# GPUs/goVideoCompressor

Hardware: AMD Instinct MI355X
Metric: encoded frames/sec (whole node), 1080p30->H.264 CRF23 (higher is better)
Workload: dtype uint8 (8-bit 4:2:0 samples, int32 transforms)

## Files before the change

csrc/kernels/bindings_hip.cc:

```cpp
#include <pybind11/pybind11.h>
#include <pybind11/stl.h>

#include <cstdint>
#include <stdexcept>
#include <vector>

#include "../common/hevc_ctu_coder.h"
#include "hevc_decode.h"
#include "route.h"

namespace py = pybind11;

extern "C" {
long long mivc_hevc_entropy_state_bytes(int W, int H);
int mivc_launch_hevc_entropy(const void* pic, int B, const int* qp, const void* ctu, const void* cu, const void* col,
                             const unsigned long long* nzmap, const int16_t* cy, const int16_t* cb, const int16_t* cr,
                             uint8_t* state, long long state_bytes, uint8_t* out, unsigned cap, unsigned* sizes,
                             int* errs, unsigned long long* offs, unsigned long long* offs_host, uint8_t* dst,
                             unsigned long long dst_cap, int* overflow, void* stream, unsigned long long* prof,
                             int* gprog, void* gctx, const unsigned long long* tsmap);
long long mivc_hevc_entropy_ctx_bytes();
int mivc_launch_hevc_tskip_probe(int nblk, const uint16_t* src, const uint16_t* pred, int16_t* lev, uint16_t* rec, int* flag,
                                 long long* terms, int bd, int qp, int intra, int dst, int scan, int sdh, int rdoq,
                                 int rdoq_lam, int lamq, void* stream);
// ... 71 lines not shown
void mivc_launch_wp_stats16(const uint16_t* y, const uint16_t* u, const uint16_t* v, int w, int h, int npics,
                            unsigned long long* out, void* stream);
void mivc_launch_wp_stats(const uint8_t* y, const uint8_t* u, const uint8_t* v, int w, int h, int npics,
                          unsigned long long* out, void* stream);
void mivc_launch_wp_src(const uint8_t* src, uint8_t* dst, const int* wt, int B, long long plane_bytes, void* stream);
void mivc_launch_p_part8(int B, int wmb, int hmb, const uint8_t* src_y, const uint8_t* ref, const uint8_t* hp,
                         const int16_t* mv, const int16_t* pm, int* cost, uint8_t* pred, int16_t* mv8, const int* qp,
                         const int8_t* aq, int overhead, int min_satd, void* stream, const void* route, int nbuf,
                         const int* bits16, const uint8_t* dir16);
void mivc_launch_encode_intra(int B, int wmb, int hmb, const uint8_t* src_y, const uint8_t* src_u,
                              const uint8_t* src_v, uint8_t* rec_y, uint8_t* rec_u, uint8_t* rec_v, const int* qp,
                              int chroma_qp_offset, void* hdr, int16_t* coef, uint8_t* nz,
                              const uint8_t* intra_flag, const int* intra_count, int* err, int use_i4x4,
                              const int8_t* aq, void* stream, int use_i8x8, const void* route, int nbuf,
                              int slice_rows, int trellis, float trellis_lambda, int* gprog, long long gprog_ints);
void mivc_launch_deblock(int B, int wmb, int hmb, uint8_t* rec_y, uint8_t* rec_u, uint8_t* rec_v, const void* hdr,
                         const uint8_t* nz, int chroma_qp_offset, int alpha_off, int beta_off, int* err,
                         void* stream, const void* route, int nbuf);
void mivc_launch_decode_picture_dpb(int B, int wmb, int hmb, int dpb_n, uint8_t* dpb_y, uint8_t* dpb_u, uint8_t* dpb_v,
                                    const int16_t* cur_idx, const int16_t* reftab, const int16_t* wp, const int16_t* sub,
                                    const void* hdr, const uint32_t* mask, const uint32_t* off,
                                    const int16_t* coef, const int8_t* run, int any_inter, int chroma_qp_offset,
                                    uint8_t* nz, int* err, void* stream);
void mivc_launch_deblock_dpb(int B, int wmb, int hmb, int dpb_n, uint8_t* dpb_y, uint8_t* dpb_u, uint8_t* dpb_v,
                             const int16_t* cur_idx, const void* hdr, const uint8_t* nz, const uint8_t* bs,
                             int chroma_qp_offset, int alpha_off, int beta_off, int* err, void* stream);
void mivc_launch_decode_picture_dpb16(int B, int wmb, int hmb, int dpb_n, uint16_t* dpb_y, uint16_t* dpb_u,
                                      uint16_t* dpb_v, const int16_t* cur_idx, const int16_t* reftab, const int16_t* wp,
                                      const int16_t* sub, const void* hdr, const uint32_t* mask, const uint32_t* off,
                                      const int16_t* coef, const int8_t* run, int any_inter, int chroma_qp_offset, int bd,
                                      uint8_t* nz, int* err, void* stream);
void mivc_launch_deblock_dpb16(int B, int wmb, int hmb, int dpb_n, uint16_t* dpb_y, uint16_t* dpb_u, uint16_t* dpb_v,
                               const int16_t* cur_idx, const void* hdr, const uint8_t* bs, int chroma_qp_offset,
// ... 377 lines not shown
                           uintptr_t ru, uintptr_t rv, uintptr_t qp, int cqo, uintptr_t hdr, uintptr_t coef,
                           uintptr_t nz, uintptr_t intra_flag, uintptr_t intra_count, uintptr_t err, int use_i4x4,
                           uintptr_t stream, uintptr_t aq, int use_i8x8, uintptr_t route, int nbuf, int slice_rows,
                           int trellis, float trellis_lambda, uintptr_t gprog, long long gprog_ints) {
    mivc_launch_encode_intra(B, wmb, hmb, P<uint8_t>(sy), P<uint8_t>(su), P<uint8_t>(sv), P<uint8_t>(ry),
                             P<uint8_t>(ru), P<uint8_t>(rv), P<int>(qp), cqo, P<void>(hdr), P<int16_t>(coef),
                             P<uint8_t>(nz), P<uint8_t>(intra_flag), P<int>(intra_count), P<int>(err), use_i4x4,
                             P<int8_t>(aq), S(stream), use_i8x8, P<void>(route), nbuf, slice_rows, trellis,
                             trellis_lambda, P<int>(gprog), gprog_ints);
  }, py::arg("B"), py::arg("wmb"), py::arg("hmb"), py::arg("sy"), py::arg("su"), py::arg("sv"), py::arg("ry"),
     py::arg("ru"), py::arg("rv"), py::arg("qp"), py::arg("cqo"), py::arg("hdr"), py::arg("coef"), py::arg("nz"),
     py::arg("intra_flag"), py::arg("intra_count"), py::arg("err"), py::arg("use_i4x4"), py::arg("stream"),
     py::arg("aq") = 0, py::arg("use_i8x8") = 0, py::arg("route") = 0, py::arg("nbuf") = 0, py::arg("slice_rows") = 0,
     py::arg("trellis") = 0, py::arg("trellis_lambda") = 1.0f, py::arg("gprog") = 0, py::arg("gprog_ints") = 0);
  m.def("deblock", [](int B, int wmb, int hmb, uintptr_t ry, uintptr_t ru, uintptr_t rv, uintptr_t hdr, uintptr_t nz,
                      int cqo, int alpha_off, int beta_off, uintptr_t err, uintptr_t stream, uintptr_t route, int nbuf) {
    mivc_launch_deblock(B, wmb, hmb, P<uint8_t>(ry), P<uint8_t>(ru), P<uint8_t>(rv), P<void>(hdr), P<uint8_t>(nz),
                        cqo, alpha_off, beta_off, P<int>(err), S(stream), P<void>(route), nbuf);
  }, py::arg("B"), py::arg("wmb"), py::arg("hmb"), py::arg("ry"), py::arg("ru"), py::arg("rv"), py::arg("hdr"),
     py::arg("nz"), py::arg("cqo"), py::arg("alpha_off"), py::arg("beta_off"), py::arg("err"), py::arg("stream"),
     py::arg("route") = 0, py::arg("nbuf") = 0);
  m.def("decode_picture_dpb", [](int B, int wmb, int hmb, int dpb_n, uintptr_t y, uintptr_t u, uintptr_t v,
                                 uintptr_t cur_idx, uintptr_t reftab, uintptr_t wp, uintptr_t sub,
                                 uintptr_t hdr, uintptr_t mask, uintptr_t off, uintptr_t coef, uintptr_t run,
                                 int any_inter, int cqo, uintptr_t nz, uintptr_t err, uintptr_t stream) {
    if (dpb_n < 1 || dpb_n > 32767) throw std::invalid_argument("decode_picture_dpb: dpb_n must be 1..32767");
    mivc_launch_decode_picture_dpb(B, wmb, hmb, dpb_n, P<uint8_t>(y), P<uint8_t>(u), P<uint8_t>(v), P<int16_t>(cur_idx),
                                   P<int16_t>(reftab), P<int16_t>(wp), P<int16_t>(sub), P<void>(hdr),
                                   P<uint32_t>(mask), P<uint32_t>(off), P<int16_t>(coef), P<int8_t>(run), any_inter,
                                   cqo, P<uint8_t>(nz), P<int>(err), S(stream));
  });
  m.def("deblock_dpb", [](int B, int wmb, int hmb, int dpb_n, uintptr_t y, uintptr_t u, uintptr_t v, uintptr_t cur_idx,
                          uintptr_t hdr, uintptr_t nz, uintptr_t bs, int cqo, int alpha_off, int beta_off, uintptr_t err,
                          uintptr_t stream) {
    if (dpb_n < 1 || dpb_n > 32767) throw std::invalid_argument("deblock_dpb: dpb_n must be 1..32767");
    mivc_launch_deblock_dpb(B, wmb, hmb, dpb_n, P<uint8_t>(y), P<uint8_t>(u), P<uint8_t>(v), P<int16_t>(cur_idx),
// ... 437 lines not shown
```

csrc/kernels/deblock.hip:

```cpp
#include "kcommon.h"

namespace mivc {
namespace gpu {

using h264::MbHeader;

struct DeblockArgs {
  Geom g;
  uint8_t *rec_y, *rec_u, *rec_v;
  const MbHeader* hdr;
  const uint8_t* nz;
  int chroma_qp_offset;
  int alpha_off, beta_off;
  int* err;
  const uint8_t* bs_in;
  int dpb_n;
  const int16_t* cur_idx;
  const SlotRoute* rt;
  int nbuf;
};

constexpr int kDeblockWaves = 16;
constexpr int kRing = 8;
constexpr int kRingU = 4;
constexpr int LT = 20;
constexpr int CT = 12;
constexpr int kSlotWords = 24;
constexpr int kMaxCols = 480;

struct DeblockShared {
  alignas(16) uint8_t ty[LT * LT];
  alignas(16) uint8_t tc[2][CT * CT];
  alignas(16) uint32_t hdrw[3][12];
  uint32_t nzw[3][4];
  int bs[2][4][4];
  int par[2][2][2][5];
  uint32_t left_y[16];
  uint32_t left_c[2][8];
  uint32_t bot_y[4][3];
  uint32_t bot_c[2][2];
};

struct DeblockTables {
  int alpha[52], beta[52], tc0[52][3], cqp[52];
};

__device__ __forceinline__ void filt(uint32_t& P, uint32_t& Q, int bs, int alpha, int beta, int tc0, bool chroma) {
  const int p3 = __builtin_amdgcn_ubfe(P, 0, 8), p2 = __builtin_amdgcn_ubfe(P, 8, 8);
  const int p1 = __builtin_amdgcn_ubfe(P, 16, 8), p0 = __builtin_amdgcn_ubfe(P, 24, 8);
  const int q0 = __builtin_amdgcn_ubfe(Q, 0, 8), q1 = __builtin_amdgcn_ubfe(Q, 8, 8);
// ... 17 lines not shown
    const bool sp = apb && strong, sq = aqb && strong;
    np0 = sp ? (p2 + 2 * p1 + 2 * p0 + 2 * q0 + q1 + 4) >> 3 : (2 * p1 + p0 + q1 + 2) >> 2;
    np1 = sp ? (p2 + p1 + p0 + q0 + 2) >> 2 : p1;
    np2 = sp ? (2 * p3 + 3 * p2 + p1 + p0 + q0 + 4) >> 3 : p2;
    nq0 = sq ? (p1 + 2 * p0 + 2 * q0 + 2 * q1 + q2 + 4) >> 3 : (2 * q1 + q0 + p1 + 2) >> 2;
    nq1 = sq ? (p0 + q0 + q1 + q2 + 2) >> 2 : q1;
    nq2 = sq ? (2 * q3 + 3 * q2 + q1 + q0 + p0 + 4) >> 3 : q2;
  }
  if (on) {
    const int pv[4] = {p3, np2, np1, np0}, qv[4] = {nq0, nq1, nq2, q3};
    P = pack4_u8(pv);
    Q = pack4_u8(qv);
  }
}

__device__ __forceinline__ void edges4(uint32_t (&d)[5], const DeblockShared& S, int dir, int line, bool chroma,
                                       bool has_nb) {
  const int seg = chroma ? (line >> 1) : (line >> 2);
#pragma unroll
  for (int e = 0; e < 4; ++e) {
    int bs = S.bs[dir][e][seg & 3];
    if (e == 0 && !has_nb) bs = 0;
    if (chroma && (e & 1)) bs = 0;
    const int* P = S.par[dir][e == 0 ? 0 : 1][chroma ? 1 : 0];
    const int tc0 = P[2 + (bs > 0 && bs < 4 ? bs - 1 : 0)];
    filt(d[e], d[e + 1], bs, P[0], P[1], tc0, chroma);
  }
}

__global__ __launch_bounds__(64 * kDeblockWaves) void deblock_wavefront(DeblockArgs a) {
  __shared__ DeblockShared SS[kDeblockWaves][2];
  __shared__ uint32_t ringL[kDeblockWaves - 1][kRing][kSlotWords];
  __shared__ uint32_t ringB[kMaxCols][kSlotWords];
  __shared__ uint32_t ringU[kDeblockWaves][kRingU][kSlotWords];
  __shared__ int prog[kMaxRows];
  __shared__ DeblockTables T;
  const Geom& g = a.g;
  const int slot = blockIdx.x;
  if (a.rt && (a.rt[slot].kind < 0 || !(a.rt[slot].flags & SF_DEBLOCK))) return;
  for (int i = threadIdx.x; i < g.hmb; i += blockDim.x) prog[i] = 0;
  for (int i = threadIdx.x; i < 52; i += blockDim.x) {
    T.alpha[i] = h264::kAlpha[i];
    T.beta[i] = h264::kBeta[i];
    T.tc0[i][0] = h264::kTc0[i][0];
    T.tc0[i][1] = h264::kTc0[i][1];
    T.tc0[i][2] = h264::kTc0[i][2];
    T.cqp[i] = h264::kChromaQp[i];
  }
  __syncthreads();
  const int w = wave_id();
  auto opaque_lane = []() { int l = lane_id(); asm volatile("" : "+v"(l)); return l; };
  const int half = lane_id() >> 5;
  DeblockShared& S = SS[w][half];
#define DB_LANE_VALUES                                                     \
  const int lane = opaque_lane(), hl = lane & 31;                          \
  const bool is_c = hl >= 16;  \
  const int ccomp = (hl - 16) >> 3, cline = hl & 7;                        \
  const int line = is_c ? cline : hl;
  const int W = g.W, cw = g.cw(), wmb = g.wmb, hmb = g.hmb;
  const size_t pic = a.dpb_n ? static_cast<size_t>(slot) * a.dpb_n + a.cur_idx[slot]
                             : route_index(a.rt, a.nbuf, slot, RO_CUR);
  uint8_t* recy = a.rec_y + pic * g.ysize();
  uint8_t* const rcu = a.rec_u + pic * g.csize();
  uint8_t* const rcv = a.rec_v + pic * g.csize();
  const uint8_t* bs_in = a.bs_in ? a.bs_in + static_cast<size_t>(slot) * g.nmb() * 16 : nullptr;
  auto recc = [&](int c) { return c ? rcv : rcu; };
  const uint32_t* hdr32 = reinterpret_cast<const uint32_t*>(a.hdr) + static_cast<size_t>(slot) * g.nmb() * 16;
  const uint32_t* nz32 = reinterpret_cast<const uint32_t*>(a.nz) + static_cast<size_t>(slot) * g.nmb() * 4;

  auto load_inputs = [&](int x, int y, uint32_t (&v)[5]) {
    DB_LANE_VALUES
    (void)line;
    const uint8_t* a1 = recy + static_cast<size_t>(y * 16 + (hl & 15)) * W + x * 16;
    const uint8_t* a2 = a1 + 8;
    if (is_c) a1 = a2 = recc(ccomp) + static_cast<size_t>(y * 8 + cline) * cw + x * 8;
    const size_t mb = static_cast<size_t>(y) * wmb + x;
    const size_t mbt = y > 0 ? mb - wmb : mb;
    const uint32_t* a3 = hl < 12 ? hdr32 + mb * 16 + hl
                                 : (hl < 24 ? hdr32 + mbt * 16 + (hl - 12)
                                            : (hl < 28 ? nz32 + mb * 4 + (hl - 24) : nz32 + mbt * 4 + (hl - 28)));
    const uint2 q1 = *reinterpret_cast<const uint2*>(a1);
    const uint2 q2 = *reinterpret_cast<const uint2*>(a2);
    v[0] = q1.x; v[1] = q1.y; v[2] = q2.x; v[3] = q2.y;
    v[4] = *a3;
  };

  for (int yu = 2 * w; yu < hmb; yu += 2 * kDeblockWaves) {
    const int yl = yu + 1;
    const int y = half ? yl : yu;
    const bool row_ok = y < hmb;
    const bool last_row = y == hmb - 1;
    const bool has_top = y > 0;
    if (half && w < kDeblockWaves - 1 && yl >= 2 * kDeblockWaves && row_ok && (lane_id() & 31) == 0)
      row_wait_lds(prog, yl - 2 * kDeblockWaves + 1, wmb, a.err);
    uint32_t nxt[5] = {0, 0, 0, 0, 0};
    if (!half) load_inputs(0, y, nxt);
    for (int step = 0; step < wmb + 2; ++step) {
      const int x = half ? step - 2 : step;
      const bool act = row_ok && x >= 0 && x < wmb;
      DB_LANE_VALUES
      const uint32_t cur[5] = {nxt[0], nxt[1], nxt[2], nxt[3], nxt[4]};
      if (row_ok && x + 1 >= 0 && x + 1 < wmb) load_inputs(x + 1, y, nxt);
      if (act) {
        const bool has_left = x > 0, last_col = x == wmb - 1;
        {
          uint32_t* dst = hl < 12 ? &S.hdrw[0][hl]
                                  : (hl < 24 ? &S.hdrw[2][hl - 12] : (hl < 28 ? &S.nzw[0][hl - 24] : &S.nzw[2][hl - 28]));
          *dst = cur[4];
        }
        wave_sync();
        const MbHeader* HQ = reinterpret_cast<const MbHeader*>(S.hdrw[0]);
        {
          const int dir = hl >> 4, e = (hl >> 2) & 3, k = hl & 3;
          int bs = 0;
          const bool mbedge = e == 0;
          if (bs_in) {
            bs = (bs_in[(static_cast<size_t>(y) * wmb + x) * 16 + (hl >> 1)] >> ((hl & 1) * 4)) & 15;
          } else if (!mbedge || (dir == 0 ? has_left : has_top)) {
            const int pw = mbedge ? (dir == 0 ? 1 : 2) : 0;
            const MbHeader* HP = reinterpret_cast<const MbHeader*>(S.hdrw[pw]);
            const uint8_t* nzbp = reinterpret_cast<const uint8_t*>(S.nzw[pw]);
            const uint8_t* nzb0 = reinterpret_cast<const uint8_t*>(S.nzw[0]);
            const int rq = dir == 0 ? (e + 4 * k) : (k + 4 * e);
            const int rp = dir == 0 ? (mbedge ? 3 + 4 * k : e - 1 + 4 * k) : (mbedge ? k + 12 : k + 4 * (e - 1));
            const bool iq = h264::mbk_is_intra(HQ->kind), ip = h264::mbk_is_intra(HP->kind);
            if ((e & 1) && (HQ->flags & h264::MBF_T8x8)) bs = 0;
            else if (mbedge && (iq || ip)) bs = 4;
            else if (iq || ip) bs = 3;
            else if (nzbp[rp] || nzb0[rq]) bs = 2;
            else {
              const int qp_ = ((rp >> 3) & 1) * 2 + ((rp & 3) >> 1), qq_ = ((rq >> 3) & 1) * 2 + ((rq & 3) >> 1);
              bool diff = false;
#pragma unroll
              for (int l = 0; l < 2; ++l) {
                const int fp = HP->ref[l][qp_], fq = HQ->ref[l][qq_];
                if ((fp >= 0) != (fq >= 0) || (fp >= 0 && fp != fq)) {
                  diff = true;
                } else if (fp >= 0) {
                  const int dx = HP->mv[l][qp_][0] - HQ->mv[l][qq_][0], dy = HP->mv[l][qp_][1] - HQ->mv[l][qq_][1];
                  diff |= dx >= 4 || dx <= -4 || dy >= 4 || dy <= -4;
                }
              }
              bs = diff ? 1 : 0;
            }
          }
          S.bs[dir][e][k] = bs;
        }
        if (hl < 8) {
          const int dir = hl >> 2, inner = (hl >> 1) & 1, ch = hl & 1;
          const int qpq = HQ->qp;
          const int qpn = reinterpret_cast<const MbHeader*>(S.hdrw[dir == 0 ? 1 : 2])->qp;
          int qq = qpq, qn = inner ? qpq : qpn;
          if (ch) {
            qq = T.cqp[clampi(qq + a.chroma_qp_offset, 0, 51)];
            qn = T.cqp[clampi(qn + a.chroma_qp_offset, 0, 51)];
          }
          const int qpav = (qq + qn + 1) >> 1;
          const int ia = clampi(qpav + a.alpha_off, 0, 51), ib = clampi(qpav + a.beta_off, 0, 51);
          int* P = S.par[dir][inner][ch];
          P[0] = T.alpha[ia];
          P[1] = T.beta[ib];
          P[2] = T.tc0[ia][0];
          P[3] = T.tc0[ia][1];
          P[4] = T.tc0[ia][2];
        }
        if (has_top) {
          if (!half) row_wait_lds(prog, y - 1, min(x + 2, wmb), a.err);
          if (hl < kSlotWords) {
            const uint32_t v = half ? ringU[w][x % kRingU][hl]
                                    : (w == 0 ? ringB[x][hl] : ringL[w - 1][x % kRing][hl]);
            if (hl < 16) *reinterpret_cast<uint32_t*>(&S.ty[(hl >> 2) * LT + 4 + (hl & 3) * 4]) = v;
            else {
              const int c = (hl - 16) >> 2, r = ((hl - 16) >> 1) & 1, h = hl & 1;
              *reinterpret_cast<uint32_t*>(&S.tc[c][(2 + r) * CT + 4 + h * 4]) = v;
            }
          }
        }
        wave_sync();

        uint32_t d[5];
        if (!is_c) {
          d[0] = has_left ? S.left_y[hl] : 0u;
          d[1] = cur[0]; d[2] = cur[1]; d[3] = cur[2]; d[4] = cur[3];
        } else {
          d[0] = has_left ? S.left_c[ccomp][cline] : 0u;
          d[1] = cur[0]; d[2] = cur[0]; d[3] = cur[1]; d[4] = 0u;
        }
        edges4(d, S, 0, line, is_c, has_left);
        if (!is_c) {
          uint32_t* row = reinterpret_cast<uint32_t*>(&S.ty[(hl + 4) * LT]);
          row[0] = d[0]; row[1] = d[1]; row[2] = d[2]; row[3] = d[3]; row[4] = d[4];
        } else {
          uint32_t* row = reinterpret_cast<uint32_t*>(&S.tc[ccomp][(cline + 4) * CT]);
          row[0] = d[0];
          row[1] = (d[1] & 0x00FFFFFFu) | (d[2] & 0xFF000000u);
          row[2] = d[3];
        }
        wave_sync();

        {
          uint8_t* col = is_c ? &S.tc[ccomp][4 + cline] : &S.ty[4 + hl];
          const int pitch = is_c ? CT : LT;
          const int nw = is_c ? 3 : 5;
          uint32_t c[5] = {0, 0, 0, 0, 0};
#pragma unroll
          for (int k = 0; k < 5; ++k) {
            if (k < nw) {
              int v4[4];
#pragma unroll
              for (int r = 0; r < 4; ++r) v4[r] = col[(4 * k + r) * pitch];
              c[k] = pack4_u8(v4);
            }
          }
          if (is_c) { c[4] = 0; c[3] = c[2]; c[2] = c[1]; }
          edges4(c, S, 1, line, is_c, has_top);
          if (is_c) { c[1] = (c[1] & 0x00FFFFFFu) | (c[2] & 0xFF000000u); c[2] = c[3]; }
#pragma unroll
          for (int k = 0; k < 5; ++k) {
            if (k < nw && (k > 0 || has_top)) {
#pragma unroll
              for (int r = 0; r < 4; ++r) col[(4 * k + r) * pitch] = static_cast<uint8_t>(c[k] >> (8 * r));
            }
          }
        }
        wave_sync();

        {
          const int r = hl & 15;
          const bool rowok = r <= 12 || last_row;
          if (!is_c) {
            if (rowok) {
              const uint8_t* t = &S.ty[(r + 4) * LT + 4];
              uint32_t* o = reinterpret_cast<uint32_t*>(recy + static_cast<size_t>(y * 16 + r) * W + x * 16);
              const uint32_t* ti = reinterpret_cast<const uint32_t*>(t);
              o[0] = ti[0]; o[1] = ti[1]; o[2] = ti[2];
              if (last_col) o[3] = ti[3];
            }
          } else if (rowok && has_left) {
            *reinterpret_cast<uint32_t*>(recy + static_cast<size_t>(y * 16 + r) * W + x * 16 - 4) =
                *reinterpret_cast<const uint32_t*>(&S.ty[(r + 4) * LT]);
          }
          if (hl < 3) {
            if (has_top) {
              const uint32_t* ti = reinterpret_cast<const uint32_t*>(&S.ty[(1 + hl) * LT + 4]);
              uint32_t* o = reinterpret_cast<uint32_t*>(recy + static_cast<size_t>(y * 16 - 3 + hl) * W + x * 16);
              o[0] = ti[0]; o[1] = ti[1]; o[2] = ti[2]; o[3] = ti[3];
            }
          } else if (hl < 5) {
            if (has_top) {
              const int c = hl - 3;
              const uint32_t* ti = reinterpret_cast<const uint32_t*>(&S.tc[c][3 * CT + 4]);
              uint32_t* o = reinterpret_cast<uint32_t*>(recc(c) + static_cast<size_t>(y * 8 - 1) * cw + x * 8);
              o[0] = ti[0]; o[1] = ti[1];
            }
          } else if (hl >= 16) {
            const int c = (hl - 16) >> 3, rc = hl & 7;
            if (rc <= 6 || last_row) {
              const uint32_t* ti = reinterpret_cast<const uint32_t*>(&S.tc[c][(rc + 4) * CT]);
              uint32_t* o = reinterpret_cast<uint32_t*>(recc(c) + static_cast<size_t>(y * 8 + rc) * cw + x * 8);
              o[0] = ti[1];
              if (last_col) o[1] = ti[2];
              if (has_left) o[-1] = ti[0];
            }
          }
        }

        if (!last_row && hl < kSlotWords) {
          uint32_t vp, vc;
          if (hl < 16) {
            const int r = hl >> 2, k = hl & 3;
            vp = k < 3 ? S.bot_y[r][k] : *reinterpret_cast<const uint32_t*>(&S.ty[(r + 16) * LT]);
            vc = *reinterpret_cast<const uint32_t*>(&S.ty[(r + 16) * LT + 4 + 4 * k]);
          } else {
            const int c = (hl - 16) >> 2, r = ((hl - 16) >> 1) & 1, h = hl & 1;
            vp = h == 0 ? S.bot_c[c][r] : *reinterpret_cast<const uint32_t*>(&S.tc[c][(r + 10) * CT]);
            vc = *reinterpret_cast<const uint32_t*>(&S.tc[c][(r + 10) * CT + 4 + 4 * h]);
          }
// ... 13 lines not shown
            }
            if (last_col) {
              if (x >= kRing) row_wait_lds(prog, y + 1, x + 1 - kRing, a.err);
              ringL[w][x % kRing][hl] = vc;
            }
          } else {
            if (has_left) ringU[w][(x - 1) % kRingU][hl] = vp;
            if (last_col) ringU[w][x % kRingU][hl] = vc;
          }
        }
        wave_sync();
        if (!is_c) S.left_y[hl] = *reinterpret_cast<const uint32_t*>(&S.ty[(hl + 4) * LT + 16]);
        else S.left_c[ccomp][cline] = *reinterpret_cast<const uint32_t*>(&S.tc[ccomp][(cline + 4) * CT + 8]);
        if (hl < 12) S.bot_y[hl / 3][hl % 3] = *reinterpret_cast<const uint32_t*>(&S.ty[(hl / 3 + 16) * LT + 4 + 4 * (hl % 3)]);
        else if (hl < 16) { const int i = hl - 12; S.bot_c[i >> 1][i & 1] = *reinterpret_cast<const uint32_t*>(&S.tc[i >> 1][((i & 1) + 10) * CT + 4]); }
        else if (hl < 28) S.hdrw[1][hl - 16] = S.hdrw[0][hl - 16];
        else S.nzw[1][hl - 28] = S.nzw[0][hl - 28];
        wave_sync();
        __builtin_amdgcn_fence(__ATOMIC_RELEASE, "workgroup", "local");
        if (hl == 0) __hip_atomic_store(prog + y, x + 1, __ATOMIC_RELAXED, __HIP_MEMORY_SCOPE_WORKGROUP);
      }
    }
  }
}

}
}

using namespace mivc::gpu;

extern "C" void mivc_launch_deblock(int B, int wmb, int hmb, uint8_t* rec_y, uint8_t* rec_u, uint8_t* rec_v,
                                    const void* hdr, const uint8_t* nz, int chroma_qp_offset, int alpha_off,
                                    int beta_off, int* err, void* stream, const void* route, int nbuf) {
  DeblockArgs a;
  a.rt = static_cast<const SlotRoute*>(route);
  a.nbuf = nbuf;
  a.g = Geom{B, wmb, hmb, wmb * 16, hmb * 16};
  a.rec_y = rec_y;
  a.rec_u = rec_u;
  a.rec_v = rec_v;
  a.hdr = static_cast<const mivc::h264::MbHeader*>(hdr);
  a.nz = nz;
  a.chroma_qp_offset = chroma_qp_offset;
  a.alpha_off = alpha_off;
  a.beta_off = beta_off;
  a.err = err;
  a.bs_in = nullptr;
  a.dpb_n = 0;
  a.cur_idx = nullptr;
  hipLaunchKernelGGL(deblock_wavefront, dim3(B), dim3(64 * kDeblockWaves), 0, static_cast<hipStream_t>(stream), a);
}

extern "C" void mivc_launch_deblock_dpb(int B, int wmb, int hmb, int dpb_n, uint8_t* dpb_y, uint8_t* dpb_u,
                                        uint8_t* dpb_v, const int16_t* cur_idx, const void* hdr, const uint8_t* nz,
                                        const uint8_t* bs, int chroma_qp_offset, int alpha_off, int beta_off, int* err,
                                        void* stream) {
  DeblockArgs a;
  a.rt = nullptr;
  a.nbuf = 0;
  a.g = Geom{B, wmb, hmb, wmb * 16, hmb * 16};
  a.rec_y = dpb_y;
  a.rec_u = dpb_u;
  a.rec_v = dpb_v;
  a.hdr = static_cast<const mivc::h264::MbHeader*>(hdr);
  a.nz = nz;
  a.chroma_qp_offset = chroma_qp_offset;
  a.alpha_off = alpha_off;
  a.beta_off = beta_off;
  a.err = err;
  a.bs_in = bs;
  a.dpb_n = dpb_n;
  a.cur_idx = cur_idx;
  hipLaunchKernelGGL(deblock_wavefront, dim3(B), dim3(64 * kDeblockWaves), 0, static_cast<hipStream_t>(stream), a);
}
```

govideocompressor_amd/models/h264_gpu.py:

```python
from __future__ import annotations

import concurrent.futures as cf
import math
import os
import time
from dataclasses import dataclass

import numpy as np
import torch

from ..ops import native
from .gop import PicPlan, col_to_list0, dpb_frames, fixed_types, gop_plan, h264_plan

MB_HDR_BYTES = 64
NO_COST = 0x3FFFFFFF
ROUTE_DTYPE = np.dtype([("kind", "i1"), ("cur", "i1"), ("n0", "i1"), ("l1", "i1"), ("l0", "i1", (4,)),
                        ("w1", "<i2", (4,)), ("dsf", "<i2", (4,)), ("dcopy", "i1", (4,)), ("flags", "u1"),
                        ("col_l1", "i1"), ("disp", "<i2")])
assert ROUTE_DTYPE.itemsize == 32
COL_NONE = -128


def col_map_row(cur: PicPlan, col: PicPlan) -> np.ndarray:
    return np.array([[COL_NONE if m is None else m - r for r, m in enumerate(row)] for row in col_to_list0(cur, col)],
# ... 260 lines not shown
        self.src = planes()
        self.nb = params.eff_bframes()
        self.nref = params.eff_refs()
        self.nref_frames = dpb_frames(self.nref, params.eff_pyramid(), self.nb)
        self.nbuf = self.nref_frames + 2
        NB = self.nbuf
        self.rec_pool = (torch.zeros((B, NB, H, W), dtype=u8, device=dev),
                         torch.zeros((B, NB, H // 2, W // 2), dtype=u8, device=dev),
                         torch.zeros((B, NB, H // 2, W // 2), dtype=u8, device=dev))
        self.rec = [tuple(p[:, i] for p in self.rec_pool) for i in range(NB)]
        self.hp_bytes = 3 * (H + 8) * (W + 8)
        self.hp_pool = torch.empty(B * NB * self.hp_bytes + 64, dtype=u8, device=dev)
        self.hdr = [torch.zeros((B, nmb, MB_HDR_BYTES), dtype=u8, device=dev) for _ in range(2)]
        self.coef = [torch.zeros((B, nmb, COEF_PER_MB), dtype=i16, device=dev) for _ in range(2)]
        self.nz = torch.zeros((B, nmb, 16), dtype=u8, device=dev)
        self.mv = torch.zeros((B, nmb, 2), dtype=i16, device=dev)
        self.mv_tmp = torch.zeros((B, nmb, 2), dtype=i16, device=dev)
        self.mv8 = torch.zeros((B, nmb, 4, 2), dtype=i16, device=dev)
        self.prev_mv = torch.zeros((B, nmb, 2), dtype=i16, device=dev)
        self.me_cost = torch.zeros((B, nmb), dtype=i32, device=dev)
        self.intra_cost = torch.zeros((B, nmb), dtype=i32, device=dev)
        self.pred = torch.zeros((B, nmb, 256), dtype=u8, device=dev)
        self.mref = torch.zeros((B, nmb), dtype=torch.int8, device=dev)
        self.dref = torch.zeros((B, nmb, 4), dtype=torch.int8, device=dev)
        self.seed = [torch.zeros((B, nmb, 2), dtype=i16, device=dev) for _ in range(2)]
        self._slot_ar = torch.arange(B, device=dev)
        if self.nref > 1:
            K = self.nref - 1
            self.xmv = torch.zeros((K, B, nmb, 2), dtype=i16, device=dev)
            self.xcost = torch.zeros((K, B, nmb), dtype=i32, device=dev)
# ... 343 lines not shown
            self.hip.encode_intra(B, wmb, hmb, sy, su, sv, py, pu, pv, P(self.qp), cqo, P(hdr), P(coef), P(self.nz),
                                  flag_ptr, count_ptr, P(self.err), int(self.p.i4x4 and trial), s, aq,
                                  int(self.p.i8x8 and self.p.eff_t8x8() and trial), rt, NB, self.slice_rows,
                                  trellis=self.p.eff_intra_trellis(), trellis_lambda=float(self.p.trellis_lambda),
                                  gprog=P(self._intra_prog), gprog_ints=self._intra_prog.numel())
        if aq:
            with stt("qp_fixup"):
                if pre:
                    self.hip.qp_fixup(B, wmb, hmb, P(hdr), P(coef), P(self.nz), P(self.qp_flags), P(self.qp), s,
                                      self.slice_rows, pre=pre["qp_flags"], route=rt)
                else:
                    self.hip.qp_fixup(B, wmb, hmb, P(hdr), P(coef), P(self.nz), P(self.qp_flags), P(self.qp), s,
                                      self.slice_rows)
        if self.p.deblock and st["deblock"]:
            with stt("deblock"):
                self.hip.deblock(B, wmb, hmb, py, pu, pv, P(hdr), P(self.nz), cqo, 0, 0, P(self.err), s, rt, NB)
        if st["ref"]:
            with stt("halfpel"):
                self.hip.me_halfpel(B, self.W, self.H, py, hpp, s, rt, NB)
            if self.nb and st["col_dst"] is not None:
                self.col_pool.view(B * NB, self.nmb, MB_HDR_BYTES).index_copy_(
                    0, st["col_dst"], hdr.index_select(0, st["col_src"]))

    def _plans(self, F: int, cuts_h: np.ndarray, anchors_at) -> list[list[PicPlan]]:
        per_slot = (isinstance(anchors_at, (list, tuple)) and len(anchors_at) == self.B and len(anchors_at) > 0
                    and all(isinstance(a, (list, tuple, set, frozenset)) for a in anchors_at))
        common = set() if per_slot else {int(d) for d in anchors_at}
        cache: dict[str, list[PicPlan]] = {}
        plans = []
        multi = getattr(self, "_la_multi", None)
        multi_intra = getattr(self, "_la_multi_intra", None) if self.p.badapt_guard else None
# ... 807 lines not shown
```

Baseline: 17490.

## Precompute deblock boundary strengths in a parallel kernel and skip quiet edges

Boundary-strength computation moves out of the serial wavefront deblock kernel into a separate fully parallel deblock_bs kernel. That kernel writes packed bs nibbles plus a per-MB info word holding the QP and an 8-bit mask of active edges. The wavefront kernel then loads the compact bs/info words instead of header and nz words, and skips filtering and stores for edges and MBs whose mask is zero. This shortens the latency-bound wavefront critical path, at the cost of an extra launch and an extra buffer, and it adds correctness risk in the store-skipping logic.

```diff
diff --git a/csrc/kernels/bindings_hip.cc b/csrc/kernels/bindings_hip.cc
--- a/csrc/kernels/bindings_hip.cc
+++ b/csrc/kernels/bindings_hip.cc
@@ -109,9 +109,11 @@
                               const uint8_t* intra_flag, const int* intra_count, int* err, int use_i4x4,
                               const int8_t* aq, void* stream, int use_i8x8, const void* route, int nbuf,
                               int slice_rows, int trellis, float trellis_lambda, int* gprog, long long gprog_ints);
-void mivc_launch_deblock(int B, int wmb, int hmb, uint8_t* rec_y, uint8_t* rec_u, uint8_t* rec_v, const void* hdr,
-                         const uint8_t* nz, int chroma_qp_offset, int alpha_off, int beta_off, int* err,
+void mivc_launch_deblock(int B, int wmb, int hmb, uint8_t* rec_y, uint8_t* rec_u, uint8_t* rec_v, const uint8_t* bs,
+                         const uint32_t* info, int chroma_qp_offset, int alpha_off, int beta_off, int* err,
                          void* stream, const void* route, int nbuf);
+void mivc_launch_deblock_bs(int B, int wmb, int hmb, const void* hdr, const uint8_t* nz, uint8_t* bs, uint32_t* info,
+                            void* stream, const void* route);
 void mivc_launch_decode_picture_dpb(int B, int wmb, int hmb, int dpb_n, uint8_t* dpb_y, uint8_t* dpb_u, uint8_t* dpb_v,
                                     const int16_t* cur_idx, const int16_t* reftab, const int16_t* wp, const int16_t* sub,
                                     const void* hdr, const uint32_t* mask, const uint32_t* off,
@@ -519,12 +521,24 @@
      py::arg("aq") = 0, py::arg("use_i8x8") = 0, py::arg("route") = 0, py::arg("nbuf") = 0, py::arg("slice_rows") = 0,
      py::arg("trellis") = 0, py::arg("trellis_lambda") = 1.0f, py::arg("gprog") = 0, py::arg("gprog_ints") = 0);
   m.def("deblock", [](int B, int wmb, int hmb, uintptr_t ry, uintptr_t ru, uintptr_t rv, uintptr_t hdr, uintptr_t nz,
-                      int cqo, int alpha_off, int beta_off, uintptr_t err, uintptr_t stream, uintptr_t route, int nbuf) {
-    mivc_launch_deblock(B, wmb, hmb, P<uint8_t>(ry), P<uint8_t>(ru), P<uint8_t>(rv), P<void>(hdr), P<uint8_t>(nz),
+                      int cqo, int alpha_off, int beta_off, uintptr_t err, uintptr_t stream, uintptr_t route, int nbuf,
+                      uintptr_t bs, uintptr_t info) {
+    if (wmb < 1 || wmb > 480 || hmb < 1 || hmb > 272) throw std::invalid_argument("deblock: at most 480 x 272 MBs");
+    if (!bs || !info) throw std::invalid_argument("deblock: needs the bs and info buffers of deblock_bs");
+    (void)hdr;
+    (void)nz;
+    mivc_launch_deblock(B, wmb, hmb, P<uint8_t>(ry), P<uint8_t>(ru), P<uint8_t>(rv), P<uint8_t>(bs), P<uint32_t>(info),
                         cqo, alpha_off, beta_off, P<int>(err), S(stream), P<void>(route), nbuf);
   }, py::arg("B"), py::arg("wmb"), py::arg("hmb"), py::arg("ry"), py::arg("ru"), py::arg("rv"), py::arg("hdr"),
      py::arg("nz"), py::arg("cqo"), py::arg("alpha_off"), py::arg("beta_off"), py::arg("err"), py::arg("stream"),
-     py::arg("route") = 0, py::arg("nbuf") = 0);
+     py::arg("route") = 0, py::arg("nbuf") = 0, py::arg("bs") = 0, py::arg("info") = 0);
+  m.def("deblock_bs", [](int B, int wmb, int hmb, uintptr_t hdr, uintptr_t nz, uintptr_t bs, uintptr_t info,
+                         uintptr_t stream, uintptr_t route) {
+    if (!hdr || !nz || !bs || !info) throw std::invalid_argument("deblock_bs: needs hdr, nz, bs and info");
+    mivc_launch_deblock_bs(B, wmb, hmb, P<void>(hdr), P<uint8_t>(nz), P<uint8_t>(bs), P<uint32_t>(info), S(stream),
+                           P<void>(route));
+  }, py::arg("B"), py::arg("wmb"), py::arg("hmb"), py::arg("hdr"), py::arg("nz"), py::arg("bs"), py::arg("info"),
+     py::arg("stream"), py::arg("route") = 0);
   m.def("decode_picture_dpb", [](int B, int wmb, int hmb, int dpb_n, uintptr_t y, uintptr_t u, uintptr_t v,
                                  uintptr_t cur_idx, uintptr_t reftab, uintptr_t wp, uintptr_t sub,
                                  uintptr_t hdr, uintptr_t mask, uintptr_t off, uintptr_t coef, uintptr_t run,
diff --git a/csrc/kernels/deblock.hip b/csrc/kernels/deblock.hip
--- a/csrc/kernels/deblock.hip
+++ b/csrc/kernels/deblock.hip
@@ -8,16 +8,27 @@
 struct DeblockArgs {
   Geom g;
   uint8_t *rec_y, *rec_u, *rec_v;
-  const MbHeader* hdr;
-  const uint8_t* nz;
   int chroma_qp_offset;
   int alpha_off, beta_off;
   int* err;
   const uint8_t* bs_in;
+  const uint32_t* info;
+  const MbHeader* hdr;
   int dpb_n;
   const int16_t* cur_idx;
   const SlotRoute* rt;
   int nbuf;
+};
+
+constexpr int kInfoOnShift = 8;
+
+struct DeblockBsArgs {
+  Geom g;
+  const MbHeader* hdr;
+  const uint8_t* nz;
+  uint8_t* bs;
+  uint32_t* info;
+  const SlotRoute* rt;
 };
 
 constexpr int kDeblockWaves = 16;
@@ -31,9 +42,6 @@
 struct DeblockShared {
   alignas(16) uint8_t ty[LT * LT];
   alignas(16) uint8_t tc[2][CT * CT];
-  alignas(16) uint32_t hdrw[3][12];
-  uint32_t nzw[3][4];
-  int bs[2][4][4];
   int par[2][2][2][5];
   uint32_t left_y[16];
   uint32_t left_c[2][8];
@@ -81,17 +89,78 @@
   }
 }
 
-__device__ __forceinline__ void edges4(uint32_t (&d)[5], const DeblockShared& S, int dir, int line, bool chroma,
-                                       bool has_nb) {
+__device__ __forceinline__ void edges4(uint32_t (&d)[5], const DeblockShared& S, uint32_t bw0, uint32_t bw1,
+                                       uint32_t on, int dir, int line, bool chroma, bool has_nb) {
   const int seg = chroma ? (line >> 1) : (line >> 2);
 #pragma unroll
   for (int e = 0; e < 4; ++e) {
-    int bs = S.bs[dir][e][seg & 3];
+    if (!(on & (1u << e))) continue;
+    int bs = ((e < 2 ? bw0 : bw1) >> (((e & 1) * 4 + (seg & 3)) * 4)) & 15;
     if (e == 0 && !has_nb) bs = 0;
     if (chroma && (e & 1)) bs = 0;
     const int* P = S.par[dir][e == 0 ? 0 : 1][chroma ? 1 : 0];
     const int tc0 = P[2 + (bs > 0 && bs < 4 ? bs - 1 : 0)];
     filt(d[e], d[e + 1], bs, P[0], P[1], tc0, chroma);
+  }
+}
+
+constexpr int kBsThreads = 256;
+__global__ __launch_bounds__(kBsThreads) void deblock_bs(DeblockBsArgs a) {
+  const Geom& g = a.g;
+  const int slot = blockIdx.y;
+  if (a.rt && (a.rt[slot].kind < 0 || !(a.rt[slot].flags & SF_DEBLOCK))) return;
+  const int nmb = g.nmb(), wmb = g.wmb;
+  const int mb = blockIdx.x * (kBsThreads / 8) + (threadIdx.x >> 3);
+  const int t = threadIdx.x & 7, dir = t >> 2, e = t & 3;
+  const bool ok = mb < nmb;
+  const size_t smb = static_cast<size_t>(slot) * nmb + (ok ? mb : 0);
+  const MbHeader* HQ = a.hdr + smb;
+  uint32_t segs = 0;
+  if (ok) {
+    const int x = mb % wmb, y = mb / wmb;
+    const bool mbedge = e == 0;
+    const bool has_nb = !mbedge || (dir == 0 ? x > 0 : y > 0);
+    if (has_nb) {
+      const size_t sp = mbedge ? (dir == 0 ? smb - 1 : smb - wmb) : smb;
+      const MbHeader* HP = a.hdr + sp;
+      const uint8_t* nzbp = a.nz + sp * 16;
+      const uint8_t* nzb0 = a.nz + smb * 16;
+      const bool iq = h264::mbk_is_intra(HQ->kind), ip = h264::mbk_is_intra(HP->kind);
+#pragma unroll
+      for (int k = 0; k < 4; ++k) {
+        const int rq = dir == 0 ? (e + 4 * k) : (k + 4 * e);
+        const int rp = dir == 0 ? (mbedge ? 3 + 4 * k : e - 1 + 4 * k) : (mbedge ? k + 12 : k + 4 * (e - 1));
+        int bs;
+        if ((e & 1) && (HQ->flags & h264::MBF_T8x8)) bs = 0;
+        else if (mbedge && (iq || ip)) bs = 4;
+        else if (iq || ip) bs = 3;
+        else if (nzbp[rp] || nzb0[rq]) bs = 2;
+        else {
+          const int qp_ = ((rp >> 3) & 1) * 2 + ((rp & 3) >> 1), qq_ = ((rq >> 3) & 1) * 2 + ((rq & 3) >> 1);
+          bool diff = false;
+#pragma unroll
+          for (int l = 0; l < 2; ++l) {
+            const int fp = HP->ref[l][qp_], fq = HQ->ref[l][qq_];
+            if ((fp >= 0) != (fq >= 0) || (fp >= 0 && fp != fq)) {
+              diff = true;
+            } else if (fp >= 0) {
+              const int dx = HP->mv[l][qp_][0] - HQ->mv[l][qq_][0], dy = HP->mv[l][qp_][1] - HQ->mv[l][qq_][1];
+              diff |= dx >= 4 || dx <= -4 || dy >= 4 || dy <= -4;
+            }
+          }
+          bs = diff ? 1 : 0;
+        }
+        segs |= static_cast<uint32_t>(bs) << (4 * k);
+      }
+    }
+  }
+  const unsigned long long on = __ballot(segs != 0);
+  if (ok) {
+    *reinterpret_cast<uint16_t*>(a.bs + smb * 16 + t * 2) = static_cast<uint16_t>(segs);
+    if (t == 0) {
+      const uint32_t bits = static_cast<uint32_t>(on >> (lane_id() & 56)) & 255u;
+      a.info[smb] = static_cast<uint32_t>(HQ->qp & 255) | (bits << kInfoOnShift);
+    }
   }
 }
 
@@ -115,7 +184,7 @@
     T.cqp[i] = h264::kChromaQp[i];
   }
   __syncthreads();
-  const int w = wave_id();
+  const int w = __builtin_amdgcn_readfirstlane(wave_id());
   auto opaque_lane = []() { int l = lane_id(); asm volatile("" : "+v"(l)); return l; };
   const int half = lane_id() >> 5;
   DeblockShared& S = SS[w][half];
@@ -130,10 +199,12 @@
   uint8_t* recy = a.rec_y + pic * g.ysize();
   uint8_t* const rcu = a.rec_u + pic * g.csize();
   uint8_t* const rcv = a.rec_v + pic * g.csize();
-  const uint8_t* bs_in = a.bs_in ? a.bs_in + static_cast<size_t>(slot) * g.nmb() * 16 : nullptr;
   auto recc = [&](int c) { return c ? rcv : rcu; };
-  const uint32_t* hdr32 = reinterpret_cast<const uint32_t*>(a.hdr) + static_cast<size_t>(slot) * g.nmb() * 16;
-  const uint32_t* nz32 = reinterpret_cast<const uint32_t*>(a.nz) + static_cast<size_t>(slot) * g.nmb() * 4;
+  const uint32_t* bs32 = reinterpret_cast<const uint32_t*>(a.bs_in) + static_cast<size_t>(slot) * g.nmb() * 4;
+  const bool has_info = a.info != nullptr;
+  const uint32_t* info32 = has_info ? a.info + static_cast<size_t>(slot) * g.nmb()
+                                    : reinterpret_cast<const uint32_t*>(a.hdr) + static_cast<size_t>(slot) * g.nmb() * 16;
+  const int info_step = has_info ? 1 : 16, qp_shift = has_info ? 0 : 16;
 
   auto load_inputs = [&](int x, int y, uint32_t (&v)[5]) {
     DB_LANE_VALUES
@@ -143,9 +214,8 @@
     if (is_c) a1 = a2 = recc(ccomp) + static_cast<size_t>(y * 8 + cline) * cw + x * 8;
     const size_t mb = static_cast<size_t>(y) * wmb + x;
     const size_t mbt = y > 0 ? mb - wmb : mb;
-    const uint32_t* a3 = hl < 12 ? hdr32 + mb * 16 + hl
-                                 : (hl < 24 ? hdr32 + mbt * 16 + (hl - 12)
-                                            : (hl < 28 ? nz32 + mb * 4 + (hl - 24) : nz32 + mbt * 4 + (hl - 28)));
+    const size_t mbtr = y > 0 && x + 1 < wmb ? mb - wmb + 1 : mb;
+    const uint32_t* a3 = hl < 4 ? bs32 + mb * 4 + hl : info32 + (hl == 5 ? mbt : (hl == 6 ? mbtr : mb)) * info_step;
     const uint2 q1 = *reinterpret_cast<const uint2*>(a1);
     const uint2 q2 = *reinterpret_cast<const uint2*>(a2);
     v[0] = q1.x; v[1] = q1.y; v[2] = q2.x; v[3] = q2.y;
@@ -161,6 +231,8 @@
     if (half && w < kDeblockWaves - 1 && yl >= 2 * kDeblockWaves && row_ok && (lane_id() & 31) == 0)
       row_wait_lds(prog, yl - 2 * kDeblockWaves + 1, wmb, a.err);
     uint32_t nxt[5] = {0, 0, 0, 0, 0};
+    int left_qp = 0;
+    bool left_quiet = false;
     if (!half) load_inputs(0, y, nxt);
     for (int step = 0; step < wmb + 2; ++step) {
       const int x = half ? step - 2 : step;
@@ -168,55 +240,38 @@
       DB_LANE_VALUES
       const uint32_t cur[5] = {nxt[0], nxt[1], nxt[2], nxt[3], nxt[4]};
       if (row_ok && x + 1 >= 0 && x + 1 < wmb) load_inputs(x + 1, y, nxt);
+      const int rec = static_cast<int>(cur[4]);
+      const bool act_u = yu < hmb && step < wmb, act_l = yl < hmb && step >= 2;
+      uint32_t on_u, on_l;
+      if (has_info) {
+        on_u = (static_cast<uint32_t>(__builtin_amdgcn_readlane(rec, 4)) >> kInfoOnShift) & 255u;
+        on_l = (static_cast<uint32_t>(__builtin_amdgcn_readlane(rec, 36)) >> kInfoOnShift) & 255u;
+      } else {
+        on_u = on_l = 0;
+#pragma unroll
+        for (int i = 0; i < 4; ++i) {
+          const uint32_t wu = static_cast<uint32_t>(__builtin_amdgcn_readlane(rec, i));
+          const uint32_t wl = static_cast<uint32_t>(__builtin_amdgcn_readlane(rec, 32 + i));
+          on_u |= ((wu & 0xFFFFu) ? 1u : 0u) << (2 * i) | ((wu >> 16) ? 2u : 0u) << (2 * i);
+          on_l |= ((wl & 0xFFFFu) ? 1u : 0u) << (2 * i) | ((wl >> 16) ? 2u : 0u) << (2 * i);
+        }
+      }
+      if (!act_u) on_u = 0;
+      if (!act_l) on_l = 0;
+      if (step == 0) on_u &= ~1u;
+      if (step == 2) on_l &= ~1u;
+      if (yu == 0) on_u &= ~16u;
+      const uint32_t on = on_u | on_l;
+#define DB_REC(i) static_cast<uint32_t>(half ? __builtin_amdgcn_readlane(rec, 32 + (i)) : __builtin_amdgcn_readlane(rec, (i)))
+      const uint32_t bsw[4] = {DB_REC(0), DB_REC(1), DB_REC(2), DB_REC(3)};
+      const uint32_t inf_q = DB_REC(4), inf_t = DB_REC(5), inf_tr = DB_REC(6);
+      const int qpq = (inf_q >> qp_shift) & 255u, qpt = (inf_t >> qp_shift) & 255u;
+#undef DB_REC
       if (act) {
         const bool has_left = x > 0, last_col = x == wmb - 1;
-        {
-          uint32_t* dst = hl < 12 ? &S.hdrw[0][hl]
-                                  : (hl < 24 ? &S.hdrw[2][hl - 12] : (hl < 28 ? &S.nzw[0][hl - 24] : &S.nzw[2][hl - 28]));
-          *dst = cur[4];
-        }
-        wave_sync();
-        const MbHeader* HQ = reinterpret_cast<const MbHeader*>(S.hdrw[0]);
-        {
-          const int dir = hl >> 4, e = (hl >> 2) & 3, k = hl & 3;
-          int bs = 0;
-          const bool mbedge = e == 0;
-          if (bs_in) {
-            bs = (bs_in[(static_cast<size_t>(y) * wmb + x) * 16 + (hl >> 1)] >> ((hl & 1) * 4)) & 15;
-          } else if (!mbedge || (dir == 0 ? has_left : has_top)) {
-            const int pw = mbedge ? (dir == 0 ? 1 : 2) : 0;
-            const MbHeader* HP = reinterpret_cast<const MbHeader*>(S.hdrw[pw]);
-            const uint8_t* nzbp = reinterpret_cast<const uint8_t*>(S.nzw[pw]);
-            const uint8_t* nzb0 = reinterpret_cast<const uint8_t*>(S.nzw[0]);
-            const int rq = dir == 0 ? (e + 4 * k) : (k + 4 * e);
-            const int rp = dir == 0 ? (mbedge ? 3 + 4 * k : e - 1 + 4 * k) : (mbedge ? k + 12 : k + 4 * (e - 1));
-            const bool iq = h264::mbk_is_intra(HQ->kind), ip = h264::mbk_is_intra(HP->kind);
-            if ((e & 1) && (HQ->flags & h264::MBF_T8x8)) bs = 0;
-            else if (mbedge && (iq || ip)) bs = 4;
-            else if (iq || ip) bs = 3;
-            else if (nzbp[rp] || nzb0[rq]) bs = 2;
-            else {
-              const int qp_ = ((rp >> 3) & 1) * 2 + ((rp & 3) >> 1), qq_ = ((rq >> 3) & 1) * 2 + ((rq & 3) >> 1);
-              bool diff = false;
-#pragma unroll
-              for (int l = 0; l < 2; ++l) {
-                const int fp = HP->ref[l][qp_], fq = HQ->ref[l][qq_];
-                if ((fp >= 0) != (fq >= 0) || (fp >= 0 && fp != fq)) {
-                  diff = true;
-                } else if (fp >= 0) {
-                  const int dx = HP->mv[l][qp_][0] - HQ->mv[l][qq_][0], dy = HP->mv[l][qp_][1] - HQ->mv[l][qq_][1];
-                  diff |= dx >= 4 || dx <= -4 || dy >= 4 || dy <= -4;
-                }
-              }
-              bs = diff ? 1 : 0;
-            }
-          }
-          S.bs[dir][e][k] = bs;
-        }
-        if (hl < 8) {
+        if (on && hl < 8) {
           const int dir = hl >> 2, inner = (hl >> 1) & 1, ch = hl & 1;
-          const int qpq = HQ->qp;
-          const int qpn = reinterpret_cast<const MbHeader*>(S.hdrw[dir == 0 ? 1 : 2])->qp;
+          const int qpn = dir == 0 ? left_qp : qpt;
           int qq = qpq, qn = inner ? qpq : qpn;
           if (ch) {
             qq = T.cqp[clampi(qq + a.chroma_qp_offset, 0, 51)];
@@ -231,6 +286,7 @@
           P[3] = T.tc0[ia][1];
           P[4] = T.tc0[ia][2];
         }
+        left_qp = qpq;
         if (has_top) {
           if (!half) row_wait_lds(prog, y - 1, min(x + 2, wmb), a.err);
           if (hl < kSlotWords) {
@@ -253,7 +309,7 @@
           d[0] = has_left ? S.left_c[ccomp][cline] : 0u;
           d[1] = cur[0]; d[2] = cur[0]; d[3] = cur[1]; d[4] = 0u;
         }
-        edges4(d, S, 0, line, is_c, has_left);
+        if (on & 15u) edges4(d, S, bsw[0], bsw[1], on & 15u, 0, line, is_c, has_left);
         if (!is_c) {
           uint32_t* row = reinterpret_cast<uint32_t*>(&S.ty[(hl + 4) * LT]);
           row[0] = d[0]; row[1] = d[1]; row[2] = d[2]; row[3] = d[3]; row[4] = d[4];
@@ -265,7 +321,7 @@
         }
         wave_sync();
 
-        {
+        if (on >> 4) {
           uint8_t* col = is_c ? &S.tc[ccomp][4 + cline] : &S.ty[4 + hl];
           const int pitch = is_c ? CT : LT;
           const int nw = is_c ? 3 : 5;
@@ -280,7 +336,7 @@
             }
           }
           if (is_c) { c[4] = 0; c[3] = c[2]; c[2] = c[1]; }
-          edges4(c, S, 1, line, is_c, has_top);
+          edges4(c, S, bsw[2], bsw[3], on >> 4, 1, line, is_c, has_top);
           if (is_c) { c[1] = (c[1] & 0x00FFFFFFu) | (c[2] & 0xFF000000u); c[2] = c[3]; }
 #pragma unroll
           for (int k = 0; k < 5; ++k) {
@@ -293,28 +349,34 @@
         wave_sync();
 
         {
+          const uint32_t own_on = half ? on_l : on_u;
+          const bool top_quiet = ((inf_t >> kInfoOnShift) & 255u) == 0;
+          const bool tr_left_on = y > 0 && !last_col && ((inf_tr >> kInfoOnShift) & 1u);
+          const bool st_own = !has_info || own_on != 0;
+          const bool st_left = !has_info || !left_quiet || (own_on & 1u);
+          const bool st_top = !has_info || !top_quiet || tr_left_on || (own_on & 16u);
           const int r = hl & 15;
           const bool rowok = r <= 12 || last_row;
           if (!is_c) {
-            if (rowok) {
+            if (rowok && st_own) {
               const uint8_t* t = &S.ty[(r + 4) * LT + 4];
               uint32_t* o = reinterpret_cast<uint32_t*>(recy + static_cast<size_t>(y * 16 + r) * W + x * 16);
               const uint32_t* ti = reinterpret_cast<const uint32_t*>(t);
               o[0] = ti[0]; o[1] = ti[1]; o[2] = ti[2];
               if (last_col) o[3] = ti[3];
             }
-          } else if (rowok && has_left) {
+          } else if (rowok && has_left && st_left) {
             *reinterpret_cast<uint32_t*>(recy + static_cast<size_t>(y * 16 + r) * W + x * 16 - 4) =
                 *reinterpret_cast<const uint32_t*>(&S.ty[(r + 4) * LT]);
           }
           if (hl < 3) {
-            if (has_top) {
+            if (has_top && st_top) {
               const uint32_t* ti = reinterpret_cast<const uint32_t*>(&S.ty[(1 + hl) * LT + 4]);
               uint32_t* o = reinterpret_cast<uint32_t*>(recy + static_cast<size_t>(y * 16 - 3 + hl) * W + x * 16);
               o[0] = ti[0]; o[1] = ti[1]; o[2] = ti[2]; o[3] = ti[3];
             }
           } else if (hl < 5) {
-            if (has_top) {
+            if (has_top && st_top) {
               const int c = hl - 3;
               const uint32_t* ti = reinterpret_cast<const uint32_t*>(&S.tc[c][3 * CT + 4]);
               uint32_t* o = reinterpret_cast<uint32_t*>(recc(c) + static_cast<size_t>(y * 8 - 1) * cw + x * 8);
@@ -325,9 +387,9 @@
             if (rc <= 6 || last_row) {
               const uint32_t* ti = reinterpret_cast<const uint32_t*>(&S.tc[c][(rc + 4) * CT]);
               uint32_t* o = reinterpret_cast<uint32_t*>(recc(c) + static_cast<size_t>(y * 8 + rc) * cw + x * 8);
-              o[0] = ti[1];
-              if (last_col) o[1] = ti[2];
-              if (has_left) o[-1] = ti[0];
+              if (st_own) o[0] = ti[1];
+              if (last_col && st_own) o[1] = ti[2];
+              if (has_left && st_left) o[-1] = ti[0];
             }
           }
         }
@@ -371,11 +433,10 @@
         else S.left_c[ccomp][cline] = *reinterpret_cast<const uint32_t*>(&S.tc[ccomp][(cline + 4) * CT + 8]);
         if (hl < 12) S.bot_y[hl / 3][hl % 3] = *reinterpret_cast<const uint32_t*>(&S.ty[(hl / 3 + 16) * LT + 4 + 4 * (hl % 3)]);
         else if (hl < 16) { const int i = hl - 12; S.bot_c[i >> 1][i & 1] = *reinterpret_cast<const uint32_t*>(&S.tc[i >> 1][((i & 1) + 10) * CT + 4]); }
-        else if (hl < 28) S.hdrw[1][hl - 16] = S.hdrw[0][hl - 16];
-        else S.nzw[1][hl - 28] = S.nzw[0][hl - 28];
         wave_sync();
         __builtin_amdgcn_fence(__ATOMIC_RELEASE, "workgroup", "local");
         if (hl == 0) __hip_atomic_store(prog + y, x + 1, __ATOMIC_RELAXED, __HIP_MEMORY_SCOPE_WORKGROUP);
+        left_quiet = ((inf_q >> kInfoOnShift) & 255u) == 0;
       }
     }
   }
@@ -386,8 +447,22 @@
 
 using namespace mivc::gpu;
 
+extern "C" void mivc_launch_deblock_bs(int B, int wmb, int hmb, const void* hdr, const uint8_t* nz, uint8_t* bs,
+                                       uint32_t* info, void* stream, const void* route) {
+  DeblockBsArgs a;
+  a.g = Geom{B, wmb, hmb, wmb * 16, hmb * 16};
+  a.hdr = static_cast<const mivc::h264::MbHeader*>(hdr);
+  a.nz = nz;
+  a.bs = bs;
+  a.info = info;
+  a.rt = static_cast<const SlotRoute*>(route);
+  const int per = kBsThreads / 8;
+  hipLaunchKernelGGL(deblock_bs, dim3((a.g.nmb() + per - 1) / per, B), dim3(kBsThreads), 0,
+                     static_cast<hipStream_t>(stream), a);
+}
+
 extern "C" void mivc_launch_deblock(int B, int wmb, int hmb, uint8_t* rec_y, uint8_t* rec_u, uint8_t* rec_v,
-                                    const void* hdr, const uint8_t* nz, int chroma_qp_offset, int alpha_off,
+                                    const uint8_t* bs, const uint32_t* info, int chroma_qp_offset, int alpha_off,
                                     int beta_off, int* err, void* stream, const void* route, int nbuf) {
   DeblockArgs a;
   a.rt = static_cast<const SlotRoute*>(route);
@@ -396,13 +471,13 @@
   a.rec_y = rec_y;
   a.rec_u = rec_u;
   a.rec_v = rec_v;
-  a.hdr = static_cast<const mivc::h264::MbHeader*>(hdr);
-  a.nz = nz;
   a.chroma_qp_offset = chroma_qp_offset;
   a.alpha_off = alpha_off;
   a.beta_off = beta_off;
   a.err = err;
-  a.bs_in = nullptr;
+  a.bs_in = bs;
+  a.info = info;
+  a.hdr = nullptr;
   a.dpb_n = 0;
   a.cur_idx = nullptr;
   hipLaunchKernelGGL(deblock_wavefront, dim3(B), dim3(64 * kDeblockWaves), 0, static_cast<hipStream_t>(stream), a);
@@ -412,6 +487,7 @@
                                         uint8_t* dpb_v, const int16_t* cur_idx, const void* hdr, const uint8_t* nz,
                                         const uint8_t* bs, int chroma_qp_offset, int alpha_off, int beta_off, int* err,
                                         void* stream) {
+  (void)nz;
   DeblockArgs a;
   a.rt = nullptr;
   a.nbuf = 0;
@@ -419,13 +495,13 @@
   a.rec_y = dpb_y;
   a.rec_u = dpb_u;
   a.rec_v = dpb_v;
-  a.hdr = static_cast<const mivc::h264::MbHeader*>(hdr);
-  a.nz = nz;
   a.chroma_qp_offset = chroma_qp_offset;
   a.alpha_off = alpha_off;
   a.beta_off = beta_off;
   a.err = err;
   a.bs_in = bs;
+  a.info = nullptr;
+  a.hdr = static_cast<const mivc::h264::MbHeader*>(hdr);
   a.dpb_n = dpb_n;
   a.cur_idx = cur_idx;
   hipLaunchKernelGGL(deblock_wavefront, dim3(B), dim3(64 * kDeblockWaves), 0, static_cast<hipStream_t>(stream), a);
diff --git a/govideocompressor_amd/models/h264_gpu.py b/govideocompressor_amd/models/h264_gpu.py
--- a/govideocompressor_amd/models/h264_gpu.py
+++ b/govideocompressor_amd/models/h264_gpu.py
@@ -298,6 +298,10 @@
         self.hdr = [torch.zeros((B, nmb, MB_HDR_BYTES), dtype=u8, device=dev) for _ in range(2)]
         self.coef = [torch.zeros((B, nmb, COEF_PER_MB), dtype=i16, device=dev) for _ in range(2)]
         self.nz = torch.zeros((B, nmb, 16), dtype=u8, device=dev)
+        self.dbk_bs = self.dbk_info = None
+        if hasattr(self.hip, "deblock_bs"):
+            self.dbk_bs = torch.zeros((B, nmb, 16), dtype=u8, device=dev)
+            self.dbk_info = torch.zeros((B, nmb), dtype=i32, device=dev)
         self.mv = torch.zeros((B, nmb, 2), dtype=i16, device=dev)
         self.mv_tmp = torch.zeros((B, nmb, 2), dtype=i16, device=dev)
         self.mv8 = torch.zeros((B, nmb, 4, 2), dtype=i16, device=dev)
@@ -671,7 +675,11 @@
                                       self.slice_rows)
         if self.p.deblock and st["deblock"]:
             with stt("deblock"):
-                self.hip.deblock(B, wmb, hmb, py, pu, pv, P(hdr), P(self.nz), cqo, 0, 0, P(self.err), s, rt, NB)
+                dkw = {}
+                if self.dbk_bs is not None:
+                    dkw = dict(bs=P(self.dbk_bs), info=P(self.dbk_info))
+                    self.hip.deblock_bs(B, wmb, hmb, P(hdr), P(self.nz), dkw["bs"], dkw["info"], s, rt)
+                self.hip.deblock(B, wmb, hmb, py, pu, pv, P(hdr), P(self.nz), cqo, 0, 0, P(self.err), s, rt, NB, **dkw)
         if st["ref"]:
             with stt("halfpel"):
                 self.hip.me_halfpel(B, self.W, self.H, py, hpp, s, rt, NB)
```

New measurement: 17690, median of 6. 1.01x the previous value.
